# pnotp/ArcFlow

Hardware: AMD Instinct MI355X
Metric: 1024x1024 images/sec @ 2 NFE (FLUX-12B architecture, denoiser + ArcFlow integrator) (higher is better)
Workload: dtype bf16; 1 GPU; ArcFlow-FLUX-12B 2-NFE inference, 1024x1024, bs=1 per GPU; nfe=2, parallelism=1 independent replica(s), no collective, lora=merged into base weights

## Files before the change

### arcflow_amd/csrc/afx_engine.hip

```cpp
#include <hip/hip_runtime.h>

#include <cstdarg>
#include <cstdio>
#include <cstring>
#include <string>
#include <unordered_map>
#include <vector>

#include "afx_api_util.h"
#include "afx_gemm_problem.h"

using namespace afx;

thread_local char afx_g_err[512] = "";

int afx_fail(int code, const char* fmt, ...) {
  va_list ap;
  va_start(ap, fmt);
  vsnprintf(afx_g_err, sizeof(afx_g_err), fmt, ap);
  va_end(ap);
  return code;
}

namespace {
// ... 5 lines not shown
};

inline int64_t align256(int64_t x) { return (x + 255) / 256 * 256; }

}

struct LinW {
  const uint16_t* w = nullptr;
  const uint16_t* b = nullptr;
  const void* wq = nullptr;
  const float* wscale = nullptr;
};
struct DoubleW { LinW qkv[2], out[2], mlp1[2], mlp2[2]; const float* qkn = nullptr; };
struct SingleW { LinW fused, out; const float* qkn = nullptr; };
struct OuterW { LinW t1, t2, g1, g2, p1, p2, mod, mod_final, x_in, ctx_in, head; const float* txt_norm = nullptr; };

struct afx_ctx {
  afx_model_desc d;
  std::unordered_map<std::string, Weight> w;
  bool finalized = false;
  std::vector<DoubleW> dbl;
  std::vector<SingleW> sgl;
  OuterW ow;
  char* ws = nullptr;
  int64_t ws_bytes = 0;
  int D = 0;
  int64_t n_mod = 0;
  int head_n = 0;
  uint16_t* ckpt = nullptr;
  bool fp8 = false;
  int fp8_mx = -1;
  const float* temb_override = nullptr;
  int prep_steps = 0, prep_B = 0, prep_use = -1;
  bool prof_on = false;
  int prof_stride = 1;
  uint64_t prof_count = 0;
  struct ProfRec { hipEvent_t a, b; int klass; double flops; };
  std::vector<ProfRec> prof_pool;
  size_t prof_used = 0;
};

namespace {

template <class T>
const T* wptr(const afx_ctx* c, const std::string& n) {
  auto it = c->w.find(n);
  return it == c->w.end() ? nullptr : (const T*)it->second.ptr;
}

int need(const afx_ctx* c, const std::string& n, int dtype, std::vector<int64_t> shape) {
  auto it = c->w.find(n);
  if (it == c->w.end()) return fail(AFX_E_MISSING, "weight '%s' is not bound", n.c_str());
  if (it->second.dtype != dtype) return fail(AFX_E_INVALID, "weight '%s': wrong dtype", n.c_str());
  if (it->second.shape != shape) {
    std::string got, want;
    for (auto v : it->second.shape) got += std::to_string(v) + ",";
    for (auto v : shape) want += std::to_string(v) + ",";
    return fail(AFX_E_INVALID, "weight '%s': shape [%s] expected [%s]", n.c_str(), got.c_str(), want.c_str());
  }
  return AFX_OK;
}

int need_linear(const afx_ctx* c, const std::string& n, int64_t out_f, int64_t in_f) {
  int r = need(c, n + ".weight", AFX_DT_BF16, {out_f, in_f});
  if (r) return r;
  return need(c, n + ".bias", AFX_DT_BF16, {out_f});
}

struct ModLayout {
  int64_t D;
  int nd, ns;
  int64_t dbl(int i, int stream , int chunk ) const {
    return ((int64_t)i * 12 + stream * 6 + chunk) * D;
  }
  int64_t sgl(int i, int chunk ) const { return (int64_t)nd * 12 * D + ((int64_t)i * 3 + chunk) * D; }
  int64_t fin(int chunk ) const { return (int64_t)nd * 12 * D + (int64_t)ns * 3 * D + chunk * D; }
  int64_t total() const { return (int64_t)nd * 12 * D + (int64_t)ns * 3 * D + 2 * D; }
};

constexpr int AFX_PREP_ROWS = 8;

struct Workspace {
  uint16_t *X, *Xn, *F, *Vt, *head;
  float *sincos, *tmp, *temb, *semb, *mod, *pooled;
  float *prep_temb, *prep_semb, *prep_mod;
  uint8_t* q8;
  uint8_t* q8n;
  uint8_t* mxn;
  uint8_t* mxw;
  float* ones;
  int64_t ld_mxn, ld_mxw;
  float* qs;
  int64_t total;
};

Workspace carve(const afx_ctx* c, char* base, int B, int N, int T) {
  const int64_t D = c->D, S = (int64_t)N + T, R = (int64_t)B * S;
  Workspace w;
  int64_t off = 0;
  auto take = [&](int64_t bytes) {
    char* p = base ? base + off : nullptr;
    off += align256(bytes);
    return p;
  };
  w.prep_temb = (float*)take((int64_t)AFX_PREP_ROWS * D * 4);
  w.prep_semb = (float*)take((int64_t)AFX_PREP_ROWS * D * 4);
  w.prep_mod = (float*)take((int64_t)AFX_PREP_ROWS * c->n_mod * 4);
  w.X = (uint16_t*)take(R * D * 2);
  w.Xn = (uint16_t*)take(R * D * 2);
  w.F = (uint16_t*)take(R * 7 * D * 2);
// ... 115 lines not shown
    kqv_problems(gb, q, A, lda, lw[s], QKV, ldq, (int64_t)b * q.S + (s == 0 ? q.T : 0), s == 0 ? q.N : q.T, b, s == 0 ? q.T : 0, 1 << 30,
                 qkn + (s == 0 ? 0 : 2) * 128, qkn + (s == 0 ? 1 : 3) * 128, true);
}

void single_qkv_batch(GemmBatch& gb, int path, const BlockShape& q, const uint16_t* A, int64_t lda, const LinW& lw, uint16_t* F, int64_t ldf,
                      const float* qkn) {
  const int64_t D = q.D;
  const int R = q.B * q.S;
  gb.nprob = 1;
  GemmProblem& f = gb.p[0];
  linear_problem(f, A, lda, lw, 0, F, ldf, R, (int)(7 * D), (int)D);
  f.epi = EPI_GELU; f.gelu_col0 = (int)(3 * D);
  if (path == AFX_QKV_VT_PROJ) {
    gb.nprob = 0;
    kqv_problems(gb, q, A, lda, lw, F, ldf, 0, R, 0, 0, q.S, qkn, qkn + 128, false);
    GemmProblem& m = gb.p[gb.nprob++];
    linear_problem(m, A, lda, lw, 3 * D, F + 3 * D, ldf, R, (int)(4 * D), (int)D);
    m.epi = EPI_GELU; m.gelu_col0 = 0;
    for (int b = 0; b < q.B; ++b) vt_problem(gb.p[gb.nprob++], q, A + (int64_t)b * q.S * lda, lda, lw, q.Vt + (int64_t)b * q.H * 128 * q.S_pad, q.S);
  } else if (path == AFX_QKV_QK_EPI) {
    set_qk_epilogue(f, q, qkn, qkn + 128, 0, q.S);
  }
}

hipError_t qkv_finish(int path, const BlockShape& q, uint16_t* F, int64_t ldf, const float* wk_txt, const float* wk_img, const float* wq_txt,
                      const float* wq_img, hipStream_t st) {
  if (path == AFX_QKV_QK_EPI) return launch_v_transpose(F + q.D, ldf, q.Vt, q.B, q.H, q.S, st);
  if (path == AFX_QKV_KV_PREP)
    return launch_kv_prep(F, F + 2 * q.D, ldf, wk_txt, wk_img, wq_txt, wq_img, q.rope_cos, q.rope_sin, q.T, F + q.D, ldf, q.Vt, q.B, q.H, q.S, st);
  return hipSuccess;
}

struct CondBufs { float *sc, *pf, *hid, *temb, *semb, *mod; };
int conditioning(const afx_ctx* c, const float* t, int nsteps, const float* g, const void* pooled, int B, const CondBufs& o, hipStream_t st) {
  const afx_model_desc& d = c->d;
  const OuterW& w = c->ow;
  const int D = c->D, rows = B * nsteps;
  for (int k = 0; k < nsteps; ++k) {
    float *hid = o.hid + (int64_t)k * B * D, *temb = o.temb + (int64_t)k * B * D;
    if (t != nullptr) {
      HIP_TRY(launch_sincos(t + (int64_t)k * B, 1000.0f, o.sc, B, d.family == 0 ? 1 : 2, st));
      HIP_TRY(launch_gemv(o.sc, w.t1.w, w.t1.b, hid, B, D, 256, 1, 0, st));
      HIP_TRY(launch_gemv(hid, w.t2.w, w.t2.b, temb, B, D, D, 0, 0, st));
    }
    if (d.guidance_embeds) {
      HIP_TRY(launch_sincos(g, 1000.0f, o.sc, B, 1, st));
      HIP_TRY(launch_gemv(o.sc, w.g1.w, w.g1.b, hid, B, D, 256, 1, 0, st));
      HIP_TRY(launch_gemv(hid, w.g2.w, w.g2.b, temb, B, D, D, 0, 1, st));
    }
    if (d.pooled_dim > 0) {
      HIP_TRY(launch_bf16_to_f32((const uint16_t*)pooled, o.pf, (int64_t)B * d.pooled_dim, st));
      HIP_TRY(launch_gemv(o.pf, w.p1.w, w.p1.b, hid, B, D, d.pooled_dim, 1, 0, st));
      HIP_TRY(launch_gemv(hid, w.p2.w, w.p2.b, temb, B, D, D, 0, 1, st));
    }
  }
  HIP_TRY(launch_silu(o.temb, o.semb, (int64_t)rows * D, st));
  HIP_TRY(launch_gemv(o.semb, w.mod.w, w.mod.b, o.mod, rows, (int)c->n_mod, D, 0, 0, st, c->n_mod));
  if (w.mod_final.w != nullptr)
    HIP_TRY(launch_gemv(o.semb, w.mod_final.w, w.mod_final.b, o.mod + ModLayout{D, d.num_double, d.num_single}.fin(0), rows, 2 * D, D, 0, 0, st, c->n_mod));
  return AFX_OK;
}

struct Fp8Mode { bool mx = false, norm_rows = false, attn_mx = false, qk_fuse_fp8 = false; };
enum class ASrc {
  Bf16,
  Wide,
  Norm,
  Attn,
};
struct Fwd {
  afx_ctx* c; Workspace ws; hipStream_t st; BlockShape bs; ModLayout ml; int64_t ldm, D, R;
  Fp8Mode fp8; int dpath, spath;
};

int fwd_gemm(Fwd& f, GemmBatch& gb) {
  ProfScope ps_(f.c, f.st, 0, gemm_flops(gb));
  HIP_TRY(launch_gemm(gb, f.st));
  return AFX_OK;
}

int fwd_resolve_fp8(Fwd& f) {
  afx_ctx* c = f.c;
  Fp8Mode& m = f.fp8;
  if (c->fp8 && c->fp8_mx < 0) {
    const char* e = getenv("AFX_FP8_MX");
    c->fp8_mx = (e && e[0] == '0') ? 0 : 1;
  }
  m.mx = c->fp8 && c->fp8_mx == 1 && f.D % 512 == 0 && gemm_fp8_mx_ok(f.R, (int)f.D, (int)f.D);
  if (m.mx) HIP_TRY(hipMemsetD32Async((hipDeviceptr_t)f.ws.ones, 0x3f800000, (size_t)f.R, f.st));
  m.norm_rows = m.mx && getenv("AFX_FP8_NORM_MX") == nullptr;
  m.attn_mx = m.mx && f.bs.H * 128 == f.D && getenv("AFX_FP8_ATTN_MX_OFF") == nullptr;
  const char* qkf8 = getenv("AFX_FP8_QK_FUSE");
  m.qk_fuse_fp8 = m.mx && qkf8 != nullptr && qkf8[0] == '1';
  f.dpath = qkv_path(f.bs, false, c->fp8, m.qk_fuse_fp8);
  f.spath = qkv_path(f.bs, true, c->fp8, m.qk_fuse_fp8);
  return AFX_OK;
}

void bind_fp8_operand(GemmProblem& p, const Fwd& f, ASrc src, int64_t row0, int K, const LinW& lw) {
  const Workspace& ws = f.ws;
  if (!f.c->fp8) return;
  p.W = (const uint16_t*)lw.wq; p.lda = K;
  if (!f.fp8.mx) {
    p.A = (const uint16_t*)(ws.q8 + row0 * K); set_fp8(p, ws.qs + row0, lw.wscale);
  } else if (src == ASrc::Norm && f.fp8.norm_rows) {
    p.A = (const uint16_t*)(ws.q8n + row0 * K); set_fp8(p, ws.qs + row0, lw.wscale);
  } else if (src == ASrc::Wide) {
    p.A = (const uint16_t*)(ws.q8 + row0 * K); set_fp8(p, ws.ones + row0, lw.wscale, ws.mxw + row0 * ws.ld_mxw, ws.ld_mxw);
  } else {
    p.A = (const uint16_t*)(ws.q8n + row0 * K); set_fp8(p, ws.ones + row0, lw.wscale, ws.mxn + row0 * ws.ld_mxn, ws.ld_mxn);
  }
}
void bind_fp8_producer(GemmProblem& p, const Fwd& f, int64_t row0, int64_t ld8, int64_t dst_col0, int col0) {
  p.c8 = f.ws.q8 + row0 * ld8 + dst_col0; p.ldc8 = ld8; p.c8_col0 = col0;
  p.c_mx = f.ws.mxw + row0 * f.ws.ld_mxw + dst_col0 / 128; p.ld_cmx = f.ws.ld_mxw;
}
int fwd_quant_operand(Fwd& f, ASrc src, const uint16_t* A, int64_t lda, int K) {
  const Workspace& ws = f.ws;
  if (f.fp8.mx && src == ASrc::Bf16) HIP_TRY(launch_quant_rows_mx8(A, lda, ws.q8n, K, ws.mxn, ws.ld_mxn, (int)f.R, K, f.st));
  else if (f.c->fp8 && !f.fp8.mx) HIP_TRY(launch_quant_rows_fp8(A, lda, ws.q8, K, ws.qs, (int)f.R, K, f.st));
  return AFX_OK;
}

int stream_gemm(Fwd& f, const uint16_t* A, int64_t lda, int K, const LinW (&lw)[2], uint16_t* C, int64_t ldc, int Nout, int epi, int blk,
                int gate_chunk, const float* qkn = nullptr, ASrc src = ASrc::Bf16, bool wide_out = false) {
  GemmBatch gb{};
  AFX_TRY(fwd_quant_operand(f, src, A, lda, K));
  for (int b = 0; b < f.bs.B; ++b)
    for (int s = 0; s < 2; ++s) {
      GemmProblem& p = gb.p[gb.nprob++];
      stream_problem(p, f.bs, A, lda, K, lw[s], C, ldc, Nout, b, s);
      const int64_t row0 = (int64_t)b * f.bs.S + (s == 0 ? f.bs.T : 0);
      bind_fp8_operand(p, f, src, row0, K, lw[s]);
      if (wide_out) bind_fp8_producer(p, f, row0, Nout, 0, 0);
      p.epi = epi;
      if (qkn != nullptr) stream_qk_epilogue(p, f.bs, qkn, s);
      if (epi == EPI_GATE_RES) set_epilogue(p, epi, 0, f.ws.mod + (int64_t)b * f.ldm + f.ml.dbl(blk, s, gate_chunk), 0, 1 << 30, C + row0 * ldc, ldc);
    }
  return fwd_gemm(f, gb);
}

int stream_norm(Fwd& f, int blk, int shift_chunk, int scale_chunk, ASrc* out) {
  const Workspace& ws = f.ws;
  const float *sc_i = ws.mod + f.ml.dbl(blk, 0, scale_chunk), *sh_i = ws.mod + f.ml.dbl(blk, 0, shift_chunk);
  const float *sc_t = ws.mod + f.ml.dbl(blk, 1, scale_chunk), *sh_t = ws.mod + f.ml.dbl(blk, 1, shift_chunk);
  bool fused = false;
  if (f.fp8.mx)
    HIP_TRY(launch_norm_modulate_mx8(ws.X, f.D, ws.q8n, f.D, ws.mxn, ws.ld_mxn, (int)f.R, (int)f.D, sc_i, sh_i, sc_t, sh_t, f.ldm, f.bs.S, f.bs.T, f.st,
                                     &fused, f.fp8.norm_rows ? ws.qs : nullptr));
  if (!fused) HIP_TRY(launch_norm_modulate_joint(ws.X, f.D, ws.Xn, f.D, (int)f.R, (int)f.D, sc_i, sh_i, sc_t, sh_t, f.ldm, f.bs.S, f.bs.T, f.st));
  *out = fused ? ASrc::Norm : ASrc::Bf16;
  return AFX_OK;
}

int fwd_conditioning(Fwd& f, const void* pooled, const float* t, const float* g) {
  afx_ctx* c = f.c;
  const Workspace& ws = f.ws;
  const int B = f.bs.B;
  const int prep_k = c->prep_use;
  c->prep_use = -1;
  if (prep_k >= 0 && prep_k < c->prep_steps && c->prep_B == B && c->temb_override == nullptr) {
    const int64_t r0 = (int64_t)prep_k * B;
    HIP_TRY(hipMemcpyAsync(ws.mod, ws.prep_mod + r0 * f.ldm, (size_t)B * f.ldm * 4, hipMemcpyDeviceToDevice, f.st));
    HIP_TRY(hipMemcpyAsync(ws.temb, ws.prep_temb + r0 * f.D, (size_t)B * f.D * 4, hipMemcpyDeviceToDevice, f.st));
    HIP_TRY(hipMemcpyAsync(ws.semb, ws.prep_semb + r0 * f.D, (size_t)B * f.D * 4, hipMemcpyDeviceToDevice, f.st));
    return AFX_OK;
  }
  if (c->temb_override != nullptr) HIP_TRY(hipMemcpyAsync(ws.temb, c->temb_override, (size_t)B * f.D * 4, hipMemcpyDeviceToDevice, f.st));
  return conditioning(c, c->temb_override != nullptr ? nullptr : t, 1, g, pooled, B, CondBufs{ws.sincos, ws.pooled, ws.tmp, ws.temb, ws.semb, ws.mod}, f.st);
}

int fwd_embed(Fwd& f, const void* x, const void* ctx_emb) {
  const afx_model_desc& d = f.c->d;
  const OuterW& w = f.c->ow;
  const Workspace& ws = f.ws;
  const int64_t B = f.bs.B, N = f.bs.N, T = f.bs.T, S = f.bs.S, D = f.D;
  const uint16_t* ctx_src = (const uint16_t*)ctx_emb;
  if (d.family == 1) {
    HIP_TRY(launch_norm_modulate(ctx_src, d.joint_dim, ws.F, d.joint_dim, (int)(B * T), d.joint_dim, w.txt_norm, nullptr, 0, (int)(B * T), 1, f.st));
    ctx_src = ws.F;
  }
  GemmBatch gb{};
  for (int b = 0; b < B; ++b) {
    linear_problem(gb.p[gb.nprob++], (const uint16_t*)x + b * N * d.in_channels, d.in_channels, w.x_in, 0, ws.X + (b * S + T) * D, D, (int)N, (int)D, d.in_channels);
    linear_problem(gb.p[gb.nprob++], ctx_src + b * T * d.joint_dim, d.joint_dim, w.ctx_in, 0, ws.X + b * S * D, D, (int)T, (int)D, d.joint_dim);
  }
  return fwd_gemm(f, gb);
}

int fwd_attention(Fwd& f, uint16_t* F, int64_t ldf, const AttnMx8& omx, bool* o_fused) {
  const BlockShape& bs = f.bs;
  ProfScope ps_(f.c, f.st, 1, 4.0 * bs.B * bs.H * (double)bs.S * bs.S * 128);
  HIP_TRY(launch_attention(F + 2 * f.D, ldf, F, ldf, f.ws.Vt, F + 2 * f.D, ldf, bs.B, bs.H, bs.S, f.st, nullptr, f.fp8.attn_mx ? &omx : nullptr, o_fused));
  return AFX_OK;
}

int fwd_double_block(Fwd& f, int i) {
  const Workspace& ws = f.ws;
  const int64_t D = f.D, R = f.R;
  const bool mx = f.fp8.mx;
  const DoubleW& bw = f.c->dbl[i];
  const float* qkn = bw.qkn;
  uint16_t* QKV = ws.F;
  uint16_t* Hb = ws.F + R * 3 * D;
  if (f.c->ckpt) HIP_TRY(hipMemcpyAsync(f.c->ckpt + (int64_t)i * R * D, ws.X, (size_t)R * D * 2, hipMemcpyDeviceToDevice, f.st));
  ASrc normed;
  AFX_TRY(stream_norm(f, i, 0, 1, &normed));
  if (f.dpath == AFX_QKV_VT_PROJ) {
    for (int b = 0; b < f.bs.B; ++b) {
      GemmBatch gb{};
      double_vt_batch(gb, f.bs, ws.Xn, D, bw.qkv, QKV, 3 * D, qkn, b);
      AFX_TRY(fwd_gemm(f, gb));
    }
  } else AFX_TRY(stream_gemm(f, ws.Xn, D, (int)D, bw.qkv, QKV, 3 * D, (int)(3 * D), EPI_NONE, i, 0, f.dpath == AFX_QKV_QK_EPI ? qkn : nullptr, normed));
  HIP_TRY(qkv_finish(f.dpath, f.bs, QKV, 3 * D, qkn + 3 * 128, qkn + 1 * 128, qkn + 2 * 128, qkn, f.st));
  bool o_fused = false;
  AFX_TRY(fwd_attention(f, QKV, 3 * D, AttnMx8{ws.q8n, D, ws.mxn, ws.ld_mxn}, &o_fused));
  AFX_TRY(stream_gemm(f, QKV + 2 * D, 3 * D, (int)D, bw.out, ws.X, D, (int)D, EPI_GATE_RES, i, 2, nullptr, o_fused ? ASrc::Attn : ASrc::Bf16));
  AFX_TRY(stream_norm(f, i, 3, 4, &normed));
  AFX_TRY(stream_gemm(f, ws.Xn, D, (int)D, bw.mlp1, Hb, 4 * D, (int)(4 * D), EPI_GELU, i, 0, nullptr, normed, mx));
  return stream_gemm(f, Hb, 4 * D, (int)(4 * D), bw.mlp2, ws.X, D, (int)D, EPI_GATE_RES, i, 5, nullptr, mx ? ASrc::Wide : ASrc::Bf16);
}

int fwd_single_block(Fwd& f, int i) {
  const Workspace& ws = f.ws;
  const int64_t D = f.D, R = f.R, ldm = f.ldm;
  const int S = f.bs.S;
  const bool mx = f.fp8.mx;
  const SingleW& bw = f.c->sgl[i];
  const float* qkn = bw.qkn;
  const float *scale = ws.mod + f.ml.sgl(i, 1), *shift = ws.mod + f.ml.sgl(i, 0);
  if (f.c->ckpt)
    HIP_TRY(hipMemcpyAsync(f.c->ckpt + (int64_t)(f.c->d.num_double + i) * R * D, ws.X, (size_t)R * D * 2, hipMemcpyDeviceToDevice, f.st));
  bool sgl_fused = false;
  if (mx) HIP_TRY(launch_norm_modulate_mx8(ws.X, D, ws.q8n, D, ws.mxn, ws.ld_mxn, (int)R, (int)D, scale, shift, nullptr, nullptr, ldm, S, 0, f.st,
                                           &sgl_fused, f.fp8.norm_rows ? ws.qs : nullptr));
  if (!sgl_fused) HIP_TRY(launch_norm_modulate(ws.X, D, ws.Xn, D, (int)R, (int)D, scale, shift, ldm, S, 0, f.st));
  const ASrc normed = sgl_fused ? ASrc::Norm : ASrc::Bf16;
  GemmBatch gb{};
  single_qkv_batch(gb, f.spath, f.bs, ws.Xn, D, bw.fused, ws.F, 7 * D, qkn);
  AFX_TRY(fwd_quant_operand(f, normed, ws.Xn, D, (int)D));
  bind_fp8_operand(gb.p[0], f, normed, 0, (int)D, bw.fused);
  if (mx) bind_fp8_producer(gb.p[0], f, 0, 5 * D, D, (int)(3 * D));
  AFX_TRY(fwd_gemm(f, gb));
  HIP_TRY(qkv_finish(f.spath, f.bs, ws.F, 7 * D, qkn + 128, qkn + 128, qkn, qkn, f.st));
  bool o_fused = false;
  AFX_TRY(fwd_attention(f, ws.F, 7 * D, AttnMx8{ws.q8, 5 * D, ws.mxw, ws.ld_mxw}, &o_fused));
  GemmBatch go{};
  GemmProblem& o = go.p[go.nprob++];
  linear_problem(o, ws.F + 2 * D, 7 * D, bw.out, 0, ws.X, D, (int)R, (int)D, (int)(5 * D));
  set_epilogue(o, EPI_GATE_RES, 0, ws.mod + f.ml.sgl(i, 2), ldm, S, ws.X, D);
  if (mx && !o_fused) HIP_TRY(launch_quant_rows_mx8(ws.F + 2 * D, 7 * D, ws.q8, 5 * D, ws.mxw, ws.ld_mxw, (int)R, (int)D, f.st));
  if (!mx) AFX_TRY(fwd_quant_operand(f, ASrc::Bf16, ws.F + 2 * D, 7 * D, (int)(5 * D)));
  bind_fp8_operand(o, f, ASrc::Wide, 0, (int)(5 * D), bw.out);
  return fwd_gemm(f, go);
}

int fwd_head(Fwd& f, void* means, void* logw, void* logg) {
  afx_ctx* c = f.c;
  const afx_model_desc& d = c->d;
  const Workspace& ws = f.ws;
  const int64_t B = f.bs.B, N = f.bs.N, T = f.bs.T, S = f.bs.S, D = f.D, ldm = f.ldm;
  for (int b = 0; b < B; ++b)
    HIP_TRY(launch_norm_modulate(ws.X + (b * S + T) * D, D, ws.Xn + b * N * D, D, (int)N, (int)D, ws.mod + b * ldm + f.ml.fin(0),
                                 ws.mod + b * ldm + f.ml.fin(1), 0, 1 << 30, 0, f.st));
  GemmBatch gb{};
  linear_problem(gb.p[gb.nprob++], ws.Xn, D, c->ow.head, 0, d.head_mode == 0 ? ws.head : (uint16_t*)means, c->head_n, (int)(B * N), c->head_n, (int)D);
  AFX_TRY(fwd_gemm(f, gb));
  if (d.head_mode == 0)
    HIP_TRY(launch_head_split(ws.head, c->head_n, (uint16_t*)means, (uint16_t*)logw, (uint16_t*)logg, B * N,
                              d.num_gaussians, d.in_channels, d.logweights_channels, f.st));
  return AFX_OK;
}

}

extern "C" {

const char* afx_last_error(void) { return afx_g_err; }
const char* afx_version(void) { return "arcflow_hip 0.1 (gfx950)"; }

int afx_create(const afx_model_desc* desc, afx_ctx** out) {
  if (!desc || !out) return fail(AFX_E_INVALID, "null argument");
  if (desc->head_dim != 128) return fail(AFX_E_UNSUPPORTED, "head_dim must be 128");
  if (desc->heads <= 0 || desc->num_double < 0 || desc->num_single < 0 || desc->num_gaussians < 1 ||
      desc->num_gaussians > 32)
    return fail(AFX_E_INVALID, "bad model description");
  if (desc->in_channels % 64 != 0 || desc->joint_dim % 64 != 0)
    return fail(AFX_E_UNSUPPORTED, "in_channels and joint_dim must be multiples of 64");
  afx_ctx* c = new afx_ctx();
  c->d = *desc;
  c->D = desc->heads * desc->head_dim;
  ModLayout ml{c->D, desc->num_double, desc->num_single};
  c->n_mod = ml.total();
  const int K = desc->num_gaussians, ch = desc->in_channels, lw = desc->logweights_channels;
  const int raw = desc->head_mode == 0 ? K * ch + K * lw + (K - 1) * lw : ch;
  c->head_n = (raw + 7) / 8 * 8;
  *out = c;
  return AFX_OK;
}

int afx_destroy(afx_ctx* ctx) {
  if (ctx) {
    for (auto& r : ctx->prof_pool) { (void)hipEventDestroy(r.a); (void)hipEventDestroy(r.b); }
  }
  delete ctx;
  return AFX_OK;
}

int afx_bind_weight(afx_ctx* ctx, const char* name, const void* dptr, int32_t dtype, int32_t ndim,
                    const int64_t* shape) {
  if (!ctx || !name || !dptr || ndim < 1 || ndim > 4 || !shape) return fail(AFX_E_INVALID, "bad bind_weight argument");
  if (dtype != AFX_DT_BF16 && dtype != AFX_DT_F32 && dtype != AFX_DT_FP8) return fail(AFX_E_INVALID, "bad dtype for '%s'", name);
  Weight w;
  w.ptr = dptr;
  w.dtype = dtype;
  w.shape.assign(shape, shape + ndim);
  ctx->w[name] = w;
  ctx->finalized = false;
  return AFX_OK;
}

int afx_finalize(afx_ctx* c) {
  if (!c) return fail(AFX_E_INVALID, "null ctx");
  const int64_t D = c->D;
  const afx_model_desc& d = c->d;
  AFX_TRY(need_linear(c, "x_in", D, d.in_channels));
  AFX_TRY(need_linear(c, "ctx_in", D, d.joint_dim));
  if (d.family == 1) AFX_TRY(need(c, "txt_norm.weight", AFX_DT_F32, {d.joint_dim}));
  AFX_TRY(need_linear(c, "temb.t.l1", D, 256));
  AFX_TRY(need_linear(c, "temb.t.l2", D, D));
  if (d.guidance_embeds) AFX_TRY(need_linear(c, "temb.g.l1", D, 256));
  if (d.guidance_embeds) AFX_TRY(need_linear(c, "temb.g.l2", D, D));
  if (d.pooled_dim > 0) AFX_TRY(need_linear(c, "temb.p.l1", D, d.pooled_dim));
  if (d.pooled_dim > 0) AFX_TRY(need_linear(c, "temb.p.l2", D, D));
  AFX_TRY(need_linear(c, "mod", c->n_mod, D));
  for (int i = 0; i < d.num_double; ++i) {
// ... 22 lines not shown
    const std::string p = "d" + std::to_string(i) + ".";
    for (int s = 0; s < 2; ++s) {
      const std::string q = p + (s == 0 ? "img_" : "txt_");
      c->dbl[i].qkv[s] = lin(q + "qkv"); c->dbl[i].out[s] = lin(q + "out");
      c->dbl[i].mlp1[s] = lin(q + "mlp1"); c->dbl[i].mlp2[s] = lin(q + "mlp2");
    }
    c->dbl[i].qkn = wptr<float>(c, p + "qknorm");
  }
  c->sgl.assign(d.num_single, SingleW{});
  for (int i = 0; i < d.num_single; ++i) {
    const std::string p = "s" + std::to_string(i) + ".";
    c->sgl[i].fused = lin(p + "fused"); c->sgl[i].out = lin(p + "out");
    c->sgl[i].qkn = wptr<float>(c, p + "qknorm");
  }
  c->ow = OuterW{lin("temb.t.l1"), lin("temb.t.l2"), lin("temb.g.l1"), lin("temb.g.l2"), lin("temb.p.l1"), lin("temb.p.l2"), lin("mod"),
                 lin("mod_final"), lin("x_in"), lin("ctx_in"), lin("head"), wptr<float>(c, "txt_norm.weight")};
  c->finalized = true;
  return AFX_OK;
}

int64_t afx_workspace_bytes(const afx_ctx* ctx, int32_t batch, int32_t n_img, int32_t n_txt) {
  if (!ctx || batch < 1 || n_img < 1 || n_txt < 0) return fail(AFX_E_INVALID, "bad workspace query");
  return carve(ctx, nullptr, batch, n_img, n_txt).total;
}

int afx_head_width(const afx_ctx* ctx) {
  if (!ctx) return fail(AFX_E_INVALID, "afx_head_width: null ctx");
  return ctx->head_n;
}

int afx_set_workspace(afx_ctx* ctx, void* dptr, int64_t bytes) {
  if (!ctx || !dptr || bytes <= 0) return fail(AFX_E_INVALID, "bad workspace");
  if (((uintptr_t)dptr & 255) != 0) return fail(AFX_E_INVALID, "workspace must be 256-byte aligned");
  ctx->ws = (char*)dptr;
  ctx->ws_bytes = bytes;
  ctx->prep_steps = 0;
  ctx->prep_use = -1;
  return AFX_OK;
}

int afx_mmdit_forward(afx_ctx* c, const void* x, const void* ctx_emb, const void* pooled, const float* t,
                      const float* g, const float* rope_cos, const float* rope_sin, int32_t B, int32_t N,
                      int32_t T, void* means, void* logw, void* logg, void* stream_) {
  return afx_mmdit_forward_stage(c, x, ctx_emb, pooled, t, g, rope_cos, rope_sin, B, N, T, means, logw, logg, 0, stream_);
}

int afx_mmdit_forward_stage(afx_ctx* c, const void* x, const void* ctx_emb, const void* pooled, const float* t,
                            const float* g, const float* rope_cos, const float* rope_sin, int32_t B, int32_t N,
                            int32_t T, void* means, void* logw, void* logg, int32_t stage, void* stream_) {
  if (stage < 0 || stage > 2) return fail(AFX_E_INVALID, "stage must be 0 (all), 1 (conditioning + embedders) or 2 (norm_out + head)");
  if (!c || !x || !ctx_emb || !t || !rope_cos || !rope_sin || !means)
    return fail(AFX_E_INVALID, "null argument to afx_mmdit_forward");
  if (!c->finalized) return fail(AFX_E_MISSING, "afx_finalize() has not succeeded on this context");
  const afx_model_desc& d = c->d;
  if (B < 1 || N < 1 || T < 1) return fail(AFX_E_INVALID, "bad shape: batch, N, T >= 1");
  if (B > AFX_MAX_MICRO_BATCH) {
    if (stage != 0 || c->ckpt) return fail(AFX_E_INVALID, "staged / checkpointed forward: batch must be 1..4 per call");
    const int64_t K = d.num_gaussians, Cc = d.in_channels, lw = d.logweights_channels;
    for (int b0 = 0; b0 < B; b0 += AFX_MAX_MICRO_BATCH) {
      const int nb = B - b0 < AFX_MAX_MICRO_BATCH ? B - b0 : AFX_MAX_MICRO_BATCH;
      const uint16_t* xb = (const uint16_t*)x + (int64_t)b0 * N * Cc;
      const uint16_t* cb = (const uint16_t*)ctx_emb + (int64_t)b0 * T * d.joint_dim;
      const uint16_t* pb = pooled ? (const uint16_t*)pooled + (int64_t)b0 * d.pooled_dim : nullptr;
      uint16_t* mb = (uint16_t*)means + (int64_t)b0 * N * (d.head_mode == 0 ? K * Cc : Cc);
      uint16_t* wb = logw ? (uint16_t*)logw + (int64_t)b0 * N * K * lw : nullptr;
      uint16_t* gb_ = logg ? (uint16_t*)logg + (int64_t)b0 * N * (K - 1) * lw : nullptr;
      const float* temb_all = c->temb_override;
      if (temb_all) c->temb_override = temb_all + (int64_t)b0 * c->D;
      const int rc = afx_mmdit_forward_stage(c, xb, cb, pb, t + b0, g ? g + b0 : nullptr, rope_cos, rope_sin, nb, N, T, mb, wb, gb_, 0, stream_);
      c->temb_override = temb_all;
      if (rc != AFX_OK) return rc;
    }
    return AFX_OK;
  }
  if (d.guidance_embeds && !g) return fail(AFX_E_INVALID, "guidance vector required");
  if (d.pooled_dim > 0 && !pooled) return fail(AFX_E_INVALID, "pooled projections required");
  if (d.head_mode == 0 && (!logw || !logg)) return fail(AFX_E_INVALID, "logw/logg outputs required");
  Workspace ws = carve(c, c->ws, B, N, T);
  if (!c->ws || ws.total > c->ws_bytes)
    return fail(AFX_E_WORKSPACE, "workspace too small: need %lld bytes, have %lld", (long long)ws.total, (long long)c->ws_bytes);
  Fwd f{c, ws, (hipStream_t)stream_, block_shape(d.heads, B, N, T, rope_cos, rope_sin, ws.Vt), ModLayout{c->D, d.num_double, d.num_single},
        c->n_mod, c->D, (int64_t)B * (N + T), Fp8Mode{}, 0, 0};
  if (stage != 2) {
    AFX_TRY(fwd_conditioning(f, pooled, t, g));
    AFX_TRY(fwd_embed(f, x, ctx_emb));
  }
  if (stage == 1) return AFX_OK;
  AFX_TRY(fwd_resolve_fp8(f));
  if (stage == 0) {
    for (int i = 0; i < d.num_double; ++i) AFX_TRY(fwd_double_block(f, i));
    for (int i = 0; i < d.num_single; ++i) AFX_TRY(fwd_single_block(f, i));
  }
  return fwd_head(f, means, logw, logg);
}

int afx_mmdit_prepare_steps(afx_ctx* c, const void* pooled, const float* t_steps, const float* g, int32_t B, int32_t nsteps,
                            void* stream_) {
  if (!c || !t_steps) return fail(AFX_E_INVALID, "null argument to afx_mmdit_prepare_steps");
  if (!c->finalized) return fail(AFX_E_MISSING, "afx_finalize() has not succeeded on this context");
  const afx_model_desc& d = c->d;
  if (B < 1 || nsteps < 1 || B > AFX_MAX_MICRO_BATCH || (int64_t)B * nsteps > AFX_PREP_ROWS)
    return fail(AFX_E_INVALID, "afx_mmdit_prepare_steps: batch <= 4 and batch * steps <= %d", AFX_PREP_ROWS);
  if (d.guidance_embeds && !g) return fail(AFX_E_INVALID, "guidance vector required");
  if (d.pooled_dim > 0 && !pooled) return fail(AFX_E_INVALID, "pooled projections required");
  if (c->temb_override) return fail(AFX_E_INVALID, "afx_mmdit_prepare_steps: not with a timestep-embedding override");
  Workspace ws = carve(c, c->ws, 1, 1, 1);
  if (!c->ws || ws.total > c->ws_bytes) return fail(AFX_E_WORKSPACE, "workspace not set / too small");
  c->prep_steps = 0; c->prep_use = -1;
  AFX_TRY(conditioning(c, t_steps, nsteps, g, pooled, B, CondBufs{ws.prep_mod, ws.prep_mod, ws.prep_semb, ws.prep_temb, ws.prep_semb, ws.prep_mod},
                       (hipStream_t)stream_));
  c->prep_steps = nsteps; c->prep_B = B;
  return AFX_OK;
}

int afx_mmdit_use_prepared_step(afx_ctx* c, int32_t k) {
  if (!c) return fail(AFX_E_INVALID, "null ctx");
  if (k >= c->prep_steps) return fail(AFX_E_INVALID, "afx_mmdit_use_prepared_step: step %d of %d prepared", k, c->prep_steps);
  c->prep_use = k < 0 ? -1 : k;
  return AFX_OK;
}

int afx_mmdit_import_tokens(afx_ctx* c, const void* src, int32_t batch, int32_t n_img, int32_t n_txt, void* stream) {
  if (!c || !src || !c->ws || batch < 1 || n_img < 1 || n_txt < 0) return fail(AFX_E_INVALID, "bad argument to afx_mmdit_import_tokens");
  Workspace ws = carve(c, c->ws, batch, n_img, n_txt);
  if (ws.total > c->ws_bytes)
    return fail(AFX_E_WORKSPACE, "afx_mmdit_import_tokens: shape (%d, %d, %d) needs %lld workspace bytes, have %lld", batch, n_img, n_txt,
                (long long)ws.total, (long long)c->ws_bytes);
  HIP_TRY(hipMemcpyAsync(ws.X, src, (size_t)batch * (n_img + n_txt) * c->D * 2, hipMemcpyDeviceToDevice, (hipStream_t)stream));
  return AFX_OK;
}

int afx_mmdit_export(afx_ctx* c, const char* what, void* dst, int32_t batch, int32_t n_img, int32_t n_txt, void* stream) {
  if (!c || !what || !dst || !c->ws || batch < 1 || n_img < 1 || n_txt < 0) return fail(AFX_E_INVALID, "bad argument to afx_mmdit_export");
  Workspace ws = carve(c, c->ws, batch, n_img, n_txt);
  if (ws.total > c->ws_bytes)
    return fail(AFX_E_WORKSPACE, "afx_mmdit_export: shape (%d, %d, %d) needs %lld workspace bytes, have %lld", batch, n_img, n_txt,
                (long long)ws.total, (long long)c->ws_bytes);
  const int64_t D = c->D;
  ModLayout ml{D, c->d.num_double, c->d.num_single};
  hipStream_t st = (hipStream_t)stream;
  const std::string w(what);
  if (w == "head_in") {
    HIP_TRY(hipMemcpyAsync(dst, ws.Xn, (size_t)batch * n_img * D * 2, hipMemcpyDeviceToDevice, st));
  } else if (w == "x_final") {
    for (int b = 0; b < batch; ++b)
      HIP_TRY(hipMemcpyAsync((char*)dst + (size_t)b * n_img * D * 2, ws.X + ((int64_t)b * (n_img + n_txt) + n_txt) * D,
                             (size_t)n_img * D * 2, hipMemcpyDeviceToDevice, st));
  } else if (w == "x_tokens") {
    HIP_TRY(hipMemcpyAsync(dst, ws.X, (size_t)batch * (n_img + n_txt) * D * 2, hipMemcpyDeviceToDevice, st));
  } else if (w == "temb") {
    HIP_TRY(hipMemcpyAsync(dst, ws.temb, (size_t)batch * D * 4, hipMemcpyDeviceToDevice, st));
  } else if (w == "silu_temb") {
    HIP_TRY(hipMemcpyAsync(dst, ws.semb, (size_t)batch * D * 4, hipMemcpyDeviceToDevice, st));
  } else if (w == "mod_all") {
    HIP_TRY(hipMemcpyAsync(dst, ws.mod, (size_t)batch * c->n_mod * 4, hipMemcpyDeviceToDevice, st));
  } else if (w == "mod_final") {
    for (int b = 0; b < batch; ++b)
      HIP_TRY(hipMemcpyAsync((char*)dst + (size_t)b * 2 * D * 4, ws.mod + (int64_t)b * c->n_mod + ml.fin(0), (size_t)2 * D * 4,
                             hipMemcpyDeviceToDevice, st));
  } else {
    return fail(AFX_E_INVALID, "afx_mmdit_export: unknown buffer '%s'", what);
  }
  return AFX_OK;
}

int afx_set_fp8_linear(afx_ctx* c, int32_t on) {
  if (!c) return fail(AFX_E_INVALID, "null ctx");
  if (on) {
    const int64_t D = c->D;
    int r;
    auto chk = [&](const std::string& n, int64_t out_f, int64_t in_f) -> int {
      if ((r = need(c, n + ".weight_q", AFX_DT_FP8, {out_f, in_f})) != AFX_OK) return r;
      return need(c, n + ".wscale", AFX_DT_F32, {out_f});
    };
    for (int i = 0; i < c->d.num_double; ++i)
      for (const char* s : {"img_", "txt_"}) {
        const std::string p = "d" + std::to_string(i) + "." + s;
        if ((r = chk(p + "qkv", 3 * D, D)) || (r = chk(p + "out", D, D)) || (r = chk(p + "mlp1", 4 * D, D)) || (r = chk(p + "mlp2", D, 4 * D))) return r;
      }
    for (int i = 0; i < c->d.num_single; ++i) {
      const std::string p = "s" + std::to_string(i) + ".";
      if ((r = chk(p + "fused", 7 * D, D)) || (r = chk(p + "out", D, 5 * D))) return r;
    }
  }
  c->fp8 = on != 0;
  return AFX_OK;
}

int afx_set_temb_override(afx_ctx* ctx, const float* temb_t) {
  if (!ctx) return fail(AFX_E_INVALID, "null ctx");
  ctx->temb_override = temb_t;
// ... 89 lines not shown
```

### include/arcflow_hip.h

```cpp
#ifndef ARCFLOW_HIP_H_
#define ARCFLOW_HIP_H_

#include <stddef.h>
#include <stdint.h>

#ifdef __cplusplus
extern "C" {
#endif

#define AFX_OK 0
#define AFX_MAX_MICRO_BATCH 4
#define AFX_E_INVALID (-1)
#define AFX_E_MISSING (-2)
#define AFX_E_WORKSPACE (-3)
#define AFX_E_HIP (-4)
#define AFX_E_UNSUPPORTED (-5)

#define AFX_DT_BF16 1
#define AFX_DT_F32 2
#define AFX_DT_FP8 3

typedef struct afx_ctx afx_ctx;

typedef struct afx_model_desc {
// ... 1 lines not shown
  int32_t num_double;
  int32_t num_single;
  int32_t heads;
  int32_t head_dim;
  int32_t in_channels;
  int32_t joint_dim;
  int32_t pooled_dim;
  int32_t guidance_embeds;
  int32_t num_gaussians;
  int32_t logweights_channels;
  int32_t head_mode;
} afx_model_desc;

const char* afx_last_error(void);
const char* afx_version(void);

int afx_create(const afx_model_desc* desc, afx_ctx** out);
int afx_destroy(afx_ctx* ctx);

int afx_bind_weight(afx_ctx* ctx, const char* name, const void* dptr, int32_t dtype,
                    int32_t ndim, const int64_t* shape);
int afx_finalize(afx_ctx* ctx);

int afx_head_width(const afx_ctx* ctx);

int64_t afx_workspace_bytes(const afx_ctx* ctx, int32_t batch, int32_t n_img, int32_t n_txt);
int afx_set_workspace(afx_ctx* ctx, void* dptr, int64_t bytes);

int afx_mmdit_forward(afx_ctx* ctx, const void* x, const void* ctx_emb, const void* pooled,
                      const float* t, const float* g, const float* rope_cos, const float* rope_sin,
                      int32_t batch, int32_t n_img, int32_t n_txt,
                      void* means, void* logw, void* logg, void* stream);

int afx_mmdit_prepare_steps(afx_ctx* ctx, const void* pooled, const float* t_steps, const float* g, int32_t batch, int32_t nsteps,
                            void* stream);
int afx_mmdit_use_prepared_step(afx_ctx* ctx, int32_t k);

int afx_set_checkpoint_buffer(afx_ctx* ctx, void* dptr);

int afx_profile_enable(afx_ctx* ctx, int32_t on);
int afx_profile_read(afx_ctx* ctx, int32_t klass, double* total_ms, int64_t* launches, double* flops);

int afx_arcflow_step(const float* x_in, const void* means, const void* logw, const void* logg,
                     int32_t mix_dtype, float sigma_src, float sigma_start, float sigma_end,
                     const float* sigma_vec, float eps, float* x_out,
                     int32_t batch, int32_t n_tok, int32_t K, int32_t ch, int32_t pp, void* stream);

int afx_arcflow_velocity(const void* means, const void* logw, const void* logg, int32_t mix_dtype,
                         float sigma_src, float sigma_t, const float* sigma_vec, float* u_out,
                         int32_t batch, int32_t n_tok, int32_t K, int32_t ch, int32_t pp, void* stream);


int afx_arcflow_step_dropout(const float* x_in, const void* means, const void* logw, const void* logg,
                             int32_t mix_dtype, const float* sigma_vec, const uint8_t* drop_mask, float eps,
                             float* x_out, int32_t batch, int32_t n_tok, int32_t K, int32_t ch, int32_t pp,
                             void* stream);

int afx_arcflow_backward(const float* g, const void* means, const void* logw, const void* logg, int32_t mix_dtype,
                         float sigma_src, float sigma_start, float sigma_end, const float* sigma_vec,
                         const float* gscale_vec, float gscale, float eps, float* d_means, float* d_logw,
                         float* d_logg, int32_t batch, int32_t n_tok, int32_t K, int32_t ch, int32_t pp,
                         int32_t velocity_only, int32_t accumulate, void* stream);

int afx_mse_loss(const float* pred, const float* target, float coef, float* grad, float* loss_accum, int64_t n,
                 void* stream);
int afx_euler_roll(const float* x_a, const float* u, const float* sigma_a, const float* sigma_b, float* out,
                   int32_t batch, int64_t per_sample, void* stream);
int afx_forward_diffuse_pack(const float* x0, const float* noise, const float* sigma, float* xt_f32, void* xt_bf16,
                             int32_t B, int32_t C, int32_t H, int32_t W, void* stream);
// ... 209 lines not shown
```

Baseline: 8.266 images/s.

## Overlap prepared modulation GEMV on side stream and read prepared rows in place

Splits the conditioning step into embedding and modulation. Prepared steps are now read directly from the prep buffers instead of being copied into the per-step workspace. When AFX_PREP_OVERLAP=1, only the first block's modulation rows are computed on the main stream. The remaining rows run on a side stream, and each block waits on that stream only once it reaches rows past the first block. This aims to hide the large modulation GEMV behind the first block's compute and to remove three device copies per step, at the cost of extra stream/event management and disabled joins during graph capture.

```diff
diff --git a/arcflow_amd/csrc/afx_engine.hip b/arcflow_amd/csrc/afx_engine.hip
--- a/arcflow_amd/csrc/afx_engine.hip
+++ b/arcflow_amd/csrc/afx_engine.hip
@@ -61,6 +61,12 @@
   int fp8_mx = -1;
   const float* temb_override = nullptr;
   int prep_steps = 0, prep_B = 0, prep_use = -1;
+  hipStream_t prep_stream = nullptr;
+  hipEvent_t prep_fork = nullptr, prep_done = nullptr;
+  bool prep_side_failed = false;
+  bool prep_body_pending = false;
+  int prep_mode = 0;
+  int64_t cond_row = -1;
   bool prof_on = false;
   int prof_stride = 1;
   uint64_t prof_count = 0;
@@ -105,6 +111,7 @@
   int64_t sgl(int i, int chunk ) const { return (int64_t)nd * 12 * D + ((int64_t)i * 3 + chunk) * D; }
   int64_t fin(int chunk ) const { return (int64_t)nd * 12 * D + (int64_t)ns * 3 * D + chunk * D; }
   int64_t total() const { return (int64_t)nd * 12 * D + (int64_t)ns * 3 * D + 2 * D; }
+  int64_t first_block_rows() const { return nd > 0 ? 12 * D : ns > 0 ? 3 * D : 0; }
 };
 
 constexpr int AFX_PREP_ROWS = 8;
@@ -286,7 +293,7 @@
 }
 
 struct CondBufs { float *sc, *pf, *hid, *temb, *semb, *mod; };
-int conditioning(const afx_ctx* c, const float* t, int nsteps, const float* g, const void* pooled, int B, const CondBufs& o, hipStream_t st) {
+int cond_embed(const afx_ctx* c, const float* t, int nsteps, const float* g, const void* pooled, int B, const CondBufs& o, hipStream_t st) {
   const afx_model_desc& d = c->d;
   const OuterW& w = c->ow;
   const int D = c->D, rows = B * nsteps;
@@ -309,10 +316,22 @@
     }
   }
   HIP_TRY(launch_silu(o.temb, o.semb, (int64_t)rows * D, st));
-  HIP_TRY(launch_gemv(o.semb, w.mod.w, w.mod.b, o.mod, rows, (int)c->n_mod, D, 0, 0, st, c->n_mod));
-  if (w.mod_final.w != nullptr)
+  return AFX_OK;
+}
+
+int cond_modulation(const afx_ctx* c, const CondBufs& o, int rows, int64_t r0, int64_t r1, hipStream_t st) {
+  const afx_model_desc& d = c->d;
+  const OuterW& w = c->ow;
+  const int D = c->D;
+  HIP_TRY(launch_gemv(o.semb, w.mod.w + r0 * D, w.mod.b + r0, o.mod + r0, rows, (int)(r1 - r0), D, 0, 0, st, c->n_mod));
+  if (w.mod_final.w != nullptr && r1 == c->n_mod)
     HIP_TRY(launch_gemv(o.semb, w.mod_final.w, w.mod_final.b, o.mod + ModLayout{D, d.num_double, d.num_single}.fin(0), rows, 2 * D, D, 0, 0, st, c->n_mod));
   return AFX_OK;
+}
+
+int conditioning(const afx_ctx* c, const float* t, int nsteps, const float* g, const void* pooled, int B, const CondBufs& o, hipStream_t st) {
+  AFX_TRY(cond_embed(c, t, nsteps, g, pooled, B, o, st));
+  return cond_modulation(c, o, B * nsteps, 0, c->n_mod, st);
 }
 
 struct Fp8Mode { bool mx = false, norm_rows = false, attn_mx = false, qk_fuse_fp8 = false; };
@@ -325,7 +344,49 @@
 struct Fwd {
   afx_ctx* c; Workspace ws; hipStream_t st; BlockShape bs; ModLayout ml; int64_t ldm, D, R;
   Fp8Mode fp8; int dpath, spath;
+  const float* mod = nullptr;
+  bool join_pending = false;
 };
+
+int prep_join(afx_ctx* c, hipStream_t st) {
+  if (!c->prep_body_pending) return AFX_OK;
+  hipStreamCaptureStatus cs = hipStreamCaptureStatusNone;
+  if (hipStreamIsCapturing(st, &cs) != hipSuccess || cs != hipStreamCaptureStatusNone) {
+    c->prep_body_pending = false;
+    return AFX_OK;
+  }
+  HIP_TRY(hipStreamWaitEvent(st, c->prep_done, 0));
+  return AFX_OK;
+}
+
+void prep_side_drain(afx_ctx* c) {
+  if (c->prep_body_pending) (void)hipStreamSynchronize(c->prep_stream);
+  c->prep_body_pending = false;
+}
+
+bool prep_side_init(afx_ctx* c) {
+  if (c->prep_side_failed) return false;
+  if (c->prep_stream != nullptr) return true;
+  hipStream_t s = nullptr;
+  hipEvent_t a = nullptr, b = nullptr;
+  if (hipStreamCreateWithFlags(&s, hipStreamNonBlocking) == hipSuccess && hipEventCreateWithFlags(&a, hipEventDisableTiming) == hipSuccess &&
+      hipEventCreateWithFlags(&b, hipEventDisableTiming) == hipSuccess) {
+    c->prep_stream = s; c->prep_fork = a; c->prep_done = b;
+    return true;
+  }
+  (void)hipGetLastError();
+  if (a) (void)hipEventDestroy(a);
+  if (b) (void)hipEventDestroy(b);
+  if (s) (void)hipStreamDestroy(s);
+  c->prep_side_failed = true;
+  return false;
+}
+
+int fwd_join(Fwd& f, int64_t row) {
+  if (!f.join_pending || row < f.ml.first_block_rows()) return AFX_OK;
+  f.join_pending = false;
+  return prep_join(f.c, f.st);
+}
 
 int fwd_gemm(Fwd& f, GemmBatch& gb) {
   ProfScope ps_(f.c, f.st, 0, gemm_flops(gb));
@@ -389,15 +450,15 @@
       if (wide_out) bind_fp8_producer(p, f, row0, Nout, 0, 0);
       p.epi = epi;
       if (qkn != nullptr) stream_qk_epilogue(p, f.bs, qkn, s);
-      if (epi == EPI_GATE_RES) set_epilogue(p, epi, 0, f.ws.mod + (int64_t)b * f.ldm + f.ml.dbl(blk, s, gate_chunk), 0, 1 << 30, C + row0 * ldc, ldc);
+      if (epi == EPI_GATE_RES) set_epilogue(p, epi, 0, f.mod + (int64_t)b * f.ldm + f.ml.dbl(blk, s, gate_chunk), 0, 1 << 30, C + row0 * ldc, ldc);
     }
   return fwd_gemm(f, gb);
 }
 
 int stream_norm(Fwd& f, int blk, int shift_chunk, int scale_chunk, ASrc* out) {
   const Workspace& ws = f.ws;
-  const float *sc_i = ws.mod + f.ml.dbl(blk, 0, scale_chunk), *sh_i = ws.mod + f.ml.dbl(blk, 0, shift_chunk);
-  const float *sc_t = ws.mod + f.ml.dbl(blk, 1, scale_chunk), *sh_t = ws.mod + f.ml.dbl(blk, 1, shift_chunk);
+  const float *sc_i = f.mod + f.ml.dbl(blk, 0, scale_chunk), *sh_i = f.mod + f.ml.dbl(blk, 0, shift_chunk);
+  const float *sc_t = f.mod + f.ml.dbl(blk, 1, scale_chunk), *sh_t = f.mod + f.ml.dbl(blk, 1, shift_chunk);
   bool fused = false;
   if (f.fp8.mx)
     HIP_TRY(launch_norm_modulate_mx8(ws.X, f.D, ws.q8n, f.D, ws.mxn, ws.ld_mxn, (int)f.R, (int)f.D, sc_i, sh_i, sc_t, sh_t, f.ldm, f.bs.S, f.bs.T, f.st,
@@ -405,6 +466,12 @@
   if (!fused) HIP_TRY(launch_norm_modulate_joint(ws.X, f.D, ws.Xn, f.D, (int)f.R, (int)f.D, sc_i, sh_i, sc_t, sh_t, f.ldm, f.bs.S, f.bs.T, f.st));
   *out = fused ? ASrc::Norm : ASrc::Bf16;
   return AFX_OK;
+}
+
+void fwd_bind_conditioning(Fwd& f) {
+  const afx_ctx* c = f.c;
+  f.mod = c->cond_row < 0 ? f.ws.mod : f.ws.prep_mod + c->cond_row * f.ldm;
+  f.join_pending = c->cond_row >= 0 && c->prep_body_pending;
 }
 
 int fwd_conditioning(Fwd& f, const void* pooled, const float* t, const float* g) {
@@ -414,12 +481,12 @@
   const int prep_k = c->prep_use;
   c->prep_use = -1;
   if (prep_k >= 0 && prep_k < c->prep_steps && c->prep_B == B && c->temb_override == nullptr) {
-    const int64_t r0 = (int64_t)prep_k * B;
-    HIP_TRY(hipMemcpyAsync(ws.mod, ws.prep_mod + r0 * f.ldm, (size_t)B * f.ldm * 4, hipMemcpyDeviceToDevice, f.st));
-    HIP_TRY(hipMemcpyAsync(ws.temb, ws.prep_temb + r0 * f.D, (size_t)B * f.D * 4, hipMemcpyDeviceToDevice, f.st));
-    HIP_TRY(hipMemcpyAsync(ws.semb, ws.prep_semb + r0 * f.D, (size_t)B * f.D * 4, hipMemcpyDeviceToDevice, f.st));
+    c->cond_row = (int64_t)prep_k * B;
+    fwd_bind_conditioning(f);
     return AFX_OK;
   }
+  c->cond_row = -1;
+  fwd_bind_conditioning(f);
   if (c->temb_override != nullptr) HIP_TRY(hipMemcpyAsync(ws.temb, c->temb_override, (size_t)B * f.D * 4, hipMemcpyDeviceToDevice, f.st));
   return conditioning(c, c->temb_override != nullptr ? nullptr : t, 1, g, pooled, B, CondBufs{ws.sincos, ws.pooled, ws.tmp, ws.temb, ws.semb, ws.mod}, f.st);
 }
@@ -459,6 +526,7 @@
   uint16_t* Hb = ws.F + R * 3 * D;
   if (f.c->ckpt) HIP_TRY(hipMemcpyAsync(f.c->ckpt + (int64_t)i * R * D, ws.X, (size_t)R * D * 2, hipMemcpyDeviceToDevice, f.st));
   ASrc normed;
+  AFX_TRY(fwd_join(f, f.ml.dbl(i, 0, 0)));
   AFX_TRY(stream_norm(f, i, 0, 1, &normed));
   if (f.dpath == AFX_QKV_VT_PROJ) {
     for (int b = 0; b < f.bs.B; ++b) {
@@ -483,10 +551,11 @@
   const bool mx = f.fp8.mx;
   const SingleW& bw = f.c->sgl[i];
   const float* qkn = bw.qkn;
-  const float *scale = ws.mod + f.ml.sgl(i, 1), *shift = ws.mod + f.ml.sgl(i, 0);
+  const float *scale = f.mod + f.ml.sgl(i, 1), *shift = f.mod + f.ml.sgl(i, 0);
   if (f.c->ckpt)
     HIP_TRY(hipMemcpyAsync(f.c->ckpt + (int64_t)(f.c->d.num_double + i) * R * D, ws.X, (size_t)R * D * 2, hipMemcpyDeviceToDevice, f.st));
   bool sgl_fused = false;
+  AFX_TRY(fwd_join(f, f.ml.sgl(i, 0)));
   if (mx) HIP_TRY(launch_norm_modulate_mx8(ws.X, D, ws.q8n, D, ws.mxn, ws.ld_mxn, (int)R, (int)D, scale, shift, nullptr, nullptr, ldm, S, 0, f.st,
                                            &sgl_fused, f.fp8.norm_rows ? ws.qs : nullptr));
   if (!sgl_fused) HIP_TRY(launch_norm_modulate(ws.X, D, ws.Xn, D, (int)R, (int)D, scale, shift, ldm, S, 0, f.st));
@@ -503,7 +572,7 @@
   GemmBatch go{};
   GemmProblem& o = go.p[go.nprob++];
   linear_problem(o, ws.F + 2 * D, 7 * D, bw.out, 0, ws.X, D, (int)R, (int)D, (int)(5 * D));
-  set_epilogue(o, EPI_GATE_RES, 0, ws.mod + f.ml.sgl(i, 2), ldm, S, ws.X, D);
+  set_epilogue(o, EPI_GATE_RES, 0, f.mod + f.ml.sgl(i, 2), ldm, S, ws.X, D);
   if (mx && !o_fused) HIP_TRY(launch_quant_rows_mx8(ws.F + 2 * D, 7 * D, ws.q8, 5 * D, ws.mxw, ws.ld_mxw, (int)R, (int)D, f.st));
   if (!mx) AFX_TRY(fwd_quant_operand(f, ASrc::Bf16, ws.F + 2 * D, 7 * D, (int)(5 * D)));
   bind_fp8_operand(o, f, ASrc::Wide, 0, (int)(5 * D), bw.out);
@@ -515,9 +584,10 @@
   const afx_model_desc& d = c->d;
   const Workspace& ws = f.ws;
   const int64_t B = f.bs.B, N = f.bs.N, T = f.bs.T, S = f.bs.S, D = f.D, ldm = f.ldm;
+  AFX_TRY(fwd_join(f, f.ml.fin(0)));
   for (int b = 0; b < B; ++b)
-    HIP_TRY(launch_norm_modulate(ws.X + (b * S + T) * D, D, ws.Xn + b * N * D, D, (int)N, (int)D, ws.mod + b * ldm + f.ml.fin(0),
-                                 ws.mod + b * ldm + f.ml.fin(1), 0, 1 << 30, 0, f.st));
+    HIP_TRY(launch_norm_modulate(ws.X + (b * S + T) * D, D, ws.Xn + b * N * D, D, (int)N, (int)D, f.mod + b * ldm + f.ml.fin(0),
+                                 f.mod + b * ldm + f.ml.fin(1), 0, 1 << 30, 0, f.st));
   GemmBatch gb{};
   linear_problem(gb.p[gb.nprob++], ws.Xn, D, c->ow.head, 0, d.head_mode == 0 ? ws.head : (uint16_t*)means, c->head_n, (int)(B * N), c->head_n, (int)D);
   AFX_TRY(fwd_gemm(f, gb));
@@ -557,6 +627,10 @@
 int afx_destroy(afx_ctx* ctx) {
   if (ctx) {
     for (auto& r : ctx->prof_pool) { (void)hipEventDestroy(r.a); (void)hipEventDestroy(r.b); }
+    prep_side_drain(ctx);
+    if (ctx->prep_fork) (void)hipEventDestroy(ctx->prep_fork);
+    if (ctx->prep_done) (void)hipEventDestroy(ctx->prep_done);
+    if (ctx->prep_stream) (void)hipStreamDestroy(ctx->prep_stream);
   }
   delete ctx;
   return AFX_OK;
@@ -645,6 +719,8 @@
 int afx_set_workspace(afx_ctx* ctx, void* dptr, int64_t bytes) {
   if (!ctx || !dptr || bytes <= 0) return fail(AFX_E_INVALID, "bad workspace");
   if (((uintptr_t)dptr & 255) != 0) return fail(AFX_E_INVALID, "workspace must be 256-byte aligned");
+  prep_side_drain(ctx);
+  ctx->cond_row = -1;
   ctx->ws = (char*)dptr;
   ctx->ws_bytes = bytes;
   ctx->prep_steps = 0;
@@ -697,6 +773,8 @@
   if (stage != 2) {
     AFX_TRY(fwd_conditioning(f, pooled, t, g));
     AFX_TRY(fwd_embed(f, x, ctx_emb));
+  } else {
+    fwd_bind_conditioning(f);
   }
   if (stage == 1) return AFX_OK;
   AFX_TRY(fwd_resolve_fp8(f));
@@ -720,9 +798,48 @@
   Workspace ws = carve(c, c->ws, 1, 1, 1);
   if (!c->ws || ws.total > c->ws_bytes) return fail(AFX_E_WORKSPACE, "workspace not set / too small");
   c->prep_steps = 0; c->prep_use = -1;
-  AFX_TRY(conditioning(c, t_steps, nsteps, g, pooled, B, CondBufs{ws.prep_mod, ws.prep_mod, ws.prep_semb, ws.prep_temb, ws.prep_semb, ws.prep_mod},
-                       (hipStream_t)stream_));
+  const hipStream_t st = (hipStream_t)stream_;
+  const CondBufs o{ws.prep_mod, ws.prep_mod, ws.prep_semb, ws.prep_temb, ws.prep_semb, ws.prep_mod};
+  const char* e = getenv("AFX_PREP_OVERLAP");
+  bool fork = e != nullptr && e[0] == '1';
+  if (fork) {
+    hipStreamCaptureStatus cs = hipStreamCaptureStatusNone;
+    fork = hipStreamIsCapturing(st, &cs) == hipSuccess && cs == hipStreamCaptureStatusNone && prep_side_init(c);
+  }
+  AFX_TRY(prep_join(c, st));
+  c->prep_body_pending = false;
+  c->prep_mode = AFX_PREP_NONE;
+  AFX_TRY(cond_embed(c, t_steps, nsteps, g, pooled, B, o, st));
+  const int rows = B * nsteps;
+  if (!fork) {
+    AFX_TRY(cond_modulation(c, o, rows, 0, c->n_mod, st));
+  } else {
+    const int64_t head = ModLayout{c->D, d.num_double, d.num_single}.first_block_rows();
+    AFX_TRY(cond_modulation(c, o, rows, 0, head, st));
+    HIP_TRY(hipEventRecord(c->prep_fork, st));
+    HIP_TRY(hipStreamWaitEvent(c->prep_stream, c->prep_fork, 0));
+    c->prep_body_pending = true;
+    AFX_TRY(cond_modulation(c, o, rows, head, c->n_mod, c->prep_stream));
+    HIP_TRY(hipEventRecord(c->prep_done, c->prep_stream));
+  }
+  c->prep_mode = fork ? AFX_PREP_FORKED : AFX_PREP_SERIAL;
   c->prep_steps = nsteps; c->prep_B = B;
+  return AFX_OK;
+}
+
+int afx_mmdit_prepare_mode(const afx_ctx* c) {
+  if (!c) return fail(AFX_E_INVALID, "null ctx");
+  return c->prep_mode;
+}
+
+int afx_mmdit_prepare_split(int32_t num_double, int32_t num_single, int32_t dim, int32_t batch, int32_t nsteps, int64_t* out6) {
+  if (num_double < 0 || num_single < 0 || dim < 1 || batch < 1 || nsteps < 1 || !out6) return fail(AFX_E_INVALID, "bad argument to afx_mmdit_prepare_split");
+  const ModLayout ml{dim, num_double, num_single};
+  const int64_t head = ml.first_block_rows();
+  out6[0] = 0; out6[1] = head;
+  out6[2] = head; out6[3] = ml.total() - head;
+  out6[4] = (int64_t)batch * nsteps;
+  out6[5] = ml.total();
   return AFX_OK;
 }
 
@@ -753,6 +870,11 @@
   ModLayout ml{D, c->d.num_double, c->d.num_single};
   hipStream_t st = (hipStream_t)stream;
   const std::string w(what);
+  const int64_t cr = c->cond_row;
+  const float* temb = cr < 0 ? ws.temb : ws.prep_temb + cr * D;
+  const float* semb = cr < 0 ? ws.semb : ws.prep_semb + cr * D;
+  const float* mod = cr < 0 ? ws.mod : ws.prep_mod + cr * c->n_mod;
+  if (cr >= 0 && (w == "mod_all" || w == "mod_final")) AFX_TRY(prep_join(c, st));
   if (w == "head_in") {
     HIP_TRY(hipMemcpyAsync(dst, ws.Xn, (size_t)batch * n_img * D * 2, hipMemcpyDeviceToDevice, st));
   } else if (w == "x_final") {
@@ -762,14 +884,14 @@
   } else if (w == "x_tokens") {
     HIP_TRY(hipMemcpyAsync(dst, ws.X, (size_t)batch * (n_img + n_txt) * D * 2, hipMemcpyDeviceToDevice, st));
   } else if (w == "temb") {
-    HIP_TRY(hipMemcpyAsync(dst, ws.temb, (size_t)batch * D * 4, hipMemcpyDeviceToDevice, st));
+    HIP_TRY(hipMemcpyAsync(dst, temb, (size_t)batch * D * 4, hipMemcpyDeviceToDevice, st));
   } else if (w == "silu_temb") {
-    HIP_TRY(hipMemcpyAsync(dst, ws.semb, (size_t)batch * D * 4, hipMemcpyDeviceToDevice, st));
+    HIP_TRY(hipMemcpyAsync(dst, semb, (size_t)batch * D * 4, hipMemcpyDeviceToDevice, st));
   } else if (w == "mod_all") {
-    HIP_TRY(hipMemcpyAsync(dst, ws.mod, (size_t)batch * c->n_mod * 4, hipMemcpyDeviceToDevice, st));
+    HIP_TRY(hipMemcpyAsync(dst, mod, (size_t)batch * c->n_mod * 4, hipMemcpyDeviceToDevice, st));
   } else if (w == "mod_final") {
     for (int b = 0; b < batch; ++b)
-      HIP_TRY(hipMemcpyAsync((char*)dst + (size_t)b * 2 * D * 4, ws.mod + (int64_t)b * c->n_mod + ml.fin(0), (size_t)2 * D * 4,
+      HIP_TRY(hipMemcpyAsync((char*)dst + (size_t)b * 2 * D * 4, mod + (int64_t)b * c->n_mod + ml.fin(0), (size_t)2 * D * 4,
                              hipMemcpyDeviceToDevice, st));
   } else {
     return fail(AFX_E_INVALID, "afx_mmdit_export: unknown buffer '%s'", what);
diff --git a/include/arcflow_hip.h b/include/arcflow_hip.h
--- a/include/arcflow_hip.h
+++ b/include/arcflow_hip.h
@@ -57,9 +57,14 @@
                       int32_t batch, int32_t n_img, int32_t n_txt,
                       void* means, void* logw, void* logg, void* stream);
 
+#define AFX_PREP_NONE 0
+#define AFX_PREP_SERIAL 1
+#define AFX_PREP_FORKED 2
 int afx_mmdit_prepare_steps(afx_ctx* ctx, const void* pooled, const float* t_steps, const float* g, int32_t batch, int32_t nsteps,
                             void* stream);
 int afx_mmdit_use_prepared_step(afx_ctx* ctx, int32_t k);
+int afx_mmdit_prepare_mode(const afx_ctx* ctx);
+int afx_mmdit_prepare_split(int32_t num_double, int32_t num_single, int32_t dim, int32_t batch, int32_t nsteps, int64_t* out6);
 
 int afx_set_checkpoint_buffer(afx_ctx* ctx, void* dptr);
 
```

Result: no change. 8.272 images/s, median of 4 (+0.1%).
